# yinjunbo/IS-Fusion

Hardware: AMD Instinct MI355X
Metric: nuScenes frames/sec forward (0.075 voxel), LiDAR branch voxelize+spconv->BEV (higher is better)
Workload: dtype f32 (f16x3 split-precision MFMA, fp32 accumulate); 1 GPU; BASELINE configs[1]: isfusion_0075voxel LiDAR-only branch (dynamic voxelize + DynamicVFE + 21-layer SparseEncoder -> BEV [B,512,180,180]), synthetic nuScenes-shaped 300000-pt sweeps, batch=4/GPU, random-init weights, eval BN, fp32; points_per_frame=300000, batch_per_gpu=4, parallelism=dp1, collectives=none (1 rank)

## Files before the change

include/isf_hip.h:

```cpp
#ifndef ISF_HIP_H
#define ISF_HIP_H

#include <stddef.h>
#include <stdint.h>

#ifdef __cplusplus
extern "C" {
#endif

#define ISF_OK 0
#define ISF_ERR_ARG (-1)
#define ISF_ERR_HIP (-2)
#define ISF_ERR_NOMEM (-3)
#define ISF_ERR_UNSUPPORTED (-4)
#define ISF_ERR_CAPACITY (-5)

#define ISF_REDUCE_SUM 0
#define ISF_REDUCE_MEAN 1
#define ISF_REDUCE_MAX 2

#define ISF_CONV_SUBM 0
#define ISF_CONV_SPARSE 1

typedef void* isf_stream_t;
// ... 104 lines not shown
#define ISF_CONV_MODE_R4_ISSUE 131072
#define ISF_CONV_MODE_TWO_AHEAD 262144
#define ISF_CONV_MODE_CHUNK_SPLIT 524288
size_t isf_packed_filter16_bytes(int num_taps, int c_in, int c_out);
int isf_pack_filters_f16x3(const float* filters, int num_taps, int c_in, int c_out, void* packed16,
                           isf_stream_t stream);
int isf_pack_filters_dx(const float* filters_t, int num_taps, int c_in, int c_out, void* packed16, float* room,
                        isf_stream_t stream);
int isf_pack_filters_f16x3_transposed(const float* filters_t, int num_taps, int c_in, int c_out, void* packed16,
                                      isf_stream_t stream);
int isf_f32_to_split(const float* x, size_t num_elems, void* xs, isf_stream_t stream);
int isf_split_to_f32(const void* xs, size_t num_elems, float* x, isf_stream_t stream);
int isf_f32_to_half(const float* x, size_t num_elems, void* xh, isf_stream_t stream);
int isf_half_to_f32(const void* xh, size_t num_elems, float* x, isf_stream_t stream);
int isf_sparse_conv_forward_f16x3(const void* features_split, int num_in, int c_in, const void* packed16,
                                  int num_taps, int c_out, const int32_t* nbr, int nbr_stride, int num_out,
                                  const float* scale, const float* shift, const void* residual_split, int relu,
                                  void* out_split, int mode, isf_stream_t stream);
int isf_sparse_conv_tile_order(const int32_t* nbr, int nbr_stride, int num_taps, int num_out, int c_in, int c_out,
                               int mode, int32_t* work, int32_t* order, int* num_entries, isf_stream_t stream);
int isf_sparse_conv_forward_f16x3_ordered(const void* features_split, int num_in, int c_in, const void* packed16,
                                          int num_taps, int c_out, const int32_t* nbr, int nbr_stride, int num_out,
                                          const float* scale, const float* shift, const void* residual_split, int relu,
                                          void* out_split, int mode, const int32_t* order, isf_stream_t stream);
int isf_sparse_conv_tile_table(const int32_t* nbr, int nbr_stride, int num_taps, int num_out, int c_in, int c_out,
                               int mode, int32_t* scratch, int32_t* table, int* num_ints, isf_stream_t stream);
int isf_sparse_conv_forward_f16x3_tiled(const void* features_split, int num_in, int c_in, const void* packed16,
                                        int num_taps, int c_out, const int32_t* nbr, int nbr_stride, int num_out,
                                        const float* scale, const float* shift, const void* residual_split, int relu,
                                        void* out_split, int mode, const int32_t* table, isf_stream_t stream);
int isf_sparse_conv_tile_table_host(const int32_t* work, int num_groups, int part_groups, int parts, int cus, int wgs_per_cu,
                                    int groups_per_tile, int32_t* tiles, int* fits);
int isf_sparse_conv_trace(const void* features_split, int num_in, int c_in, const void* packed16, int num_taps,
                          int c_out, const int32_t* nbr, int nbr_stride, int num_out, const float* scale,
                          const float* shift, const void* residual_split, int relu, void* out_split,
                          const int32_t* order, long long* trace, int trace_capacity_blocks, int* grid_blocks,
                          isf_stream_t stream);
int isf_sparse_conv_phase_trace(const void* features_split, int num_in, int c_in, const void* packed16, int num_taps,
                                int c_out, const int32_t* nbr, int nbr_stride, int num_out, const float* scale,
                                const float* shift, const void* residual_split, int relu, void* out_split,
                                const int32_t* order, long long* trace, size_t trace_bytes, int* grid_blocks,
                                int* waves_per_block, int* dwords_per_wave, isf_stream_t stream);

int isf_sparse_conv_dma_trace(const void* features_split, int num_in, int c_in, const void* packed16, int num_taps,
                              int taps_per_line, int c_out, const int32_t* table, const uint32_t* mask, int nbr_stride,
                              int num_out, const float* scale, const float* shift, const void* residual_split, int relu,
                              void* out_split, long long* trace, int trace_capacity_blocks, int* grid_blocks,
                              isf_stream_t stream);
int isf_sparse_conv_dma_trace_parts(const void* features_split, int num_in, int c_in, const void* packed16, int num_taps,
                                    int taps_per_line, int c_out, const int32_t* table, const uint32_t* mask, int nbr_stride,
                                    int num_out, const float* scale, const float* shift, const void* residual_split, int relu,
                                    void* out_split, const int32_t* part_table, long long* trace, int trace_capacity_blocks,
                                    int* grid_blocks, isf_stream_t stream);
int isf_sparse_conv_part_table(const int32_t* table_nbr, const uint32_t* mask, int nbr_stride, int num_taps, int num_out,
                               int c_in, int c_out, int mode, int flags, int32_t* work, int work_capacity, int32_t* part_table,
                               int table_capacity, int* info, isf_stream_t stream);
int isf_sparse_conv_forward_parts(const void* features_split, int num_in, int c_in, const void* packed16, int num_taps,
                                  int taps_per_line, int c_out, const int32_t* table_nbr, const uint32_t* mask, int nbr_stride,
                                  int num_out, const float* scale, const float* shift, const void* residual_split, int relu,
                                  void* out_split, int mode, const int32_t* part_table, isf_stream_t stream);
int isf_sparse_conv_forward_dma(const void* features_split, int num_in, int c_in, const void* packed16, int num_taps,
                                int c_out, const int32_t* nbr, int nbr_stride, int num_out, const float* scale,
                                const float* shift, const void* residual_split, int relu, void* out_split, int mode,
                                const int32_t* order, isf_stream_t stream);
int isf_rulebook_to_lines(const int32_t* nbr, int nbr_stride, int num_taps, int taps_per_line, int num_out,
                          int32_t* lines, uint32_t* mask, int* not_consecutive_flag, isf_stream_t stream);
int isf_lines_to_rulebook(const int32_t* lines, const uint32_t* mask, int nbr_stride, int num_taps, int taps_per_line,
                          int32_t* nbr, isf_stream_t stream);
int isf_sparse_conv_forward_dma_lines(const void* features_split, int num_in, int c_in, const void* packed16, int num_taps,
                                      int taps_per_line, int c_out, const int32_t* lines, const uint32_t* mask,
                                      int nbr_stride, int num_out, const float* scale, const float* shift,
                                      const void* residual_split, int relu, void* out_split, int mode,
                                      isf_stream_t stream);
typedef struct isf_conv_cu_plan {
  const int32_t* group_masks;
  const int32_t* units;
  const int32_t* num_units;
  int max_units;
  int num_out;
  int variant;
  int cap;
} isf_conv_cu_plan;
int isf_sparse_conv_cu_plan_ints(int num_out, size_t* num_ints);
int isf_sparse_conv_cu_plan(const int32_t* nbr, int nbr_stride, int num_taps, int num_out, int32_t* plan_buf,
                            isf_conv_cu_plan* plan, isf_stream_t stream);
int isf_sparse_conv_forward_cu(const void* features_split, int num_in, int c_in, const void* packed16, int num_taps,
                               int c_out, const int32_t* nbr, int nbr_stride, int num_out, const float* scale,
                               const float* shift, const void* residual_split, int relu, void* out_split,
                               const isf_conv_cu_plan* plan, isf_stream_t stream);
int isf_sparse_conv_cu_plan_host(const int32_t* work, int num_groups, int cus, int32_t* units, int max_units,
                                 int* num_units);
int isf_sparse_conv_cu_max_units(int num_groups, int cus);
int isf_stage_unit_rows(void);
int isf_stage_unit_cap(void);
int isf_rulebook_stage_tables(const int32_t* nbr, int nbr_stride, int num_taps, uint16_t* slots, int32_t* ulist,
                              int32_t* ucount, isf_stream_t stream);
int isf_sparse_conv_forward_staged(const void* features_split, int num_in, int c_in, const void* packed16,
                                   int num_taps, int c_out, const uint16_t* slots, int nbr_stride,
                                   const int32_t* ulist, const int32_t* ucount, int num_out, const float* scale,
                                   const float* shift, const void* residual_split, int relu, void* out_split,
                                   int stage_rows, int mode, isf_stream_t stream);
int isf_sparse_to_dense_bev(const float* features, const int32_t* indices, int num_rows, int channels,
                            int batch_size, int D, int H, int W, float* out, isf_stream_t stream);

typedef struct isf_conv_layer {
  int conv_type;
// ... 509 lines not shown
```

is-fusion_amd/_lib.py:

```python
import ctypes
import os

_HERE = os.path.dirname(os.path.abspath(__file__))
LIB_PATH = os.path.join(_HERE, "libisf_hip.so")

c_int = ctypes.c_int
c_void_p = ctypes.c_void_p
c_float_p = ctypes.POINTER(ctypes.c_float)
c_int_p = ctypes.POINTER(ctypes.c_int)

ISF_OK = 0
REDUCE = {"sum": 0, "mean": 1, "max": 2}
CONV_SUBM, CONV_SPARSE = 0, 1


class ConvLayer(ctypes.Structure):
    _fields_ = [
        ("conv_type", c_int),
        ("ksize", c_int * 3), ("stride", c_int * 3), ("padding", c_int * 3),
        ("c_in", c_int), ("c_out", c_int),
        ("packed", c_void_p), ("packed16", c_void_p), ("scale", c_void_p), ("shift", c_void_p),
        ("relu", c_int), ("residual_from", c_int),
    ]

# ... 216 lines not shown
    "isf_ingroup_indices": (c_int, [c_void_p, c_int, c_void_p, c_void_p]),
    "isf_packed_window_block_bytes": (ctypes.c_size_t, [c_int]),
    "isf_pack_window_block": (c_int, [c_void_p, c_void_p, c_int, c_int, c_void_p, c_void_p]),
    "isf_window_block_forward": (c_int, [c_void_p, c_int, c_int, c_int, c_int, c_int, c_int, c_void_p, c_void_p,
                                         c_void_p, c_void_p, c_void_p, c_void_p, ctypes.c_float, c_void_p, c_void_p]),
    "isf_p2g_backward": (c_int, [c_void_p, c_int, c_int, c_void_p, c_int, c_int, c_int, c_int, c_int, c_int, c_void_p,
                                 c_int, c_int, c_int, c_void_p, c_void_p, c_void_p]),
    "isf_p2g_backward_det": (c_int, [c_void_p, c_int, c_int, c_void_p, c_int, c_int, c_int, c_int, c_int, c_int, c_void_p,
                                 c_int, c_int, c_int, c_void_p, c_void_p, c_void_p]),
    "isf_sparse_to_dense_bev": (c_int, [c_void_p, c_void_p, c_int, c_int, c_int, c_int, c_int, c_int,
                                        c_void_p, c_void_p]),
    "isf_sparse_encoder_forward": (c_int, [c_void_p, c_void_p, c_int, c_int, _I3,
                                           ctypes.POINTER(ConvLayer), c_int, c_void_p, _I4,
                                           ctypes.POINTER(EncoderStats), c_int, ctypes.POINTER(EncoderOptions),
                                           c_void_p]),
    "isf_lidar_branch_forward": (c_int, [c_void_p, ctypes.POINTER(ctypes.c_int64), c_int,
                                         ctypes.POINTER(VfeParams), _I3, ctypes.POINTER(ConvLayer), c_int,
                                         c_void_p, _I4, ctypes.POINTER(EncoderStats), c_int,
                                         ctypes.POINTER(EncoderOptions), c_void_p]),
    "isf_lidar_branch_forward_frames": (c_int, [ctypes.POINTER(c_void_p), ctypes.POINTER(ctypes.c_int64), c_int,
                                                ctypes.POINTER(VfeParams), _I3, ctypes.POINTER(ConvLayer), c_int,
                                                c_void_p, _I4, ctypes.POINTER(EncoderStats), c_int,
                                                ctypes.POINTER(EncoderOptions), c_void_p]),
    "isf_packed_linear_bytes": (ctypes.c_size_t, [c_int, c_int]),
    "isf_pack_linear": (c_int, [c_void_p, c_int, c_int, c_void_p, c_void_p]),
    "isf_pack_linear_transposed": (c_int, [c_void_p, c_int, c_int, c_void_p, c_void_p]),
    "isf_linear_forward": (c_int, [c_void_p, c_int, c_int, c_int, c_void_p, c_int, c_void_p, c_void_p, c_void_p,
                                   c_int, c_void_p, c_void_p, c_void_p, ctypes.c_float, c_void_p, c_int, c_int, c_int,
                                   c_int, c_void_p]),
    "isf_window_attention_forward": (c_int, [c_void_p, c_int, c_int, c_int, c_int, c_int, c_int, c_void_p,
                                             c_void_p]),
    "isf_attention_forward": (c_int, [c_void_p, c_int, c_void_p, c_void_p, c_int, c_int, c_int, c_int, c_int,
                                      c_int, c_void_p, c_int, c_void_p]),
    "isf_attention_forward_dropout": (c_int, [c_void_p, c_int, c_void_p, c_void_p, c_int, c_int, c_int, c_int, c_int,
                                              c_int, ctypes.c_float, ctypes.c_uint64, c_void_p, c_int, c_void_p]),
    "isf_channel_attention_forward": (c_int, [c_void_p, c_void_p, c_int, c_int, c_void_p, c_void_p]),
    "isf_channel_attention_backward": (c_int, [c_void_p, c_void_p, c_void_p, c_int, c_int, c_void_p, c_void_p, c_void_p]),
    "isf_p2g_forward": (c_int, [c_void_p, c_int, c_int, c_void_p, c_int, c_void_p, c_int, c_int, c_int, c_int,
                                c_int, c_void_p, c_int, c_int, c_int, c_void_p, c_void_p]),
    "isf_p2g_forward_split": (c_int, [c_void_p, c_int, c_int, c_void_p, c_int, c_void_p, c_int, c_int, c_int, c_int,
                                      c_int, c_void_p, c_int, c_int, c_int, c_void_p, c_void_p]),
    "isf_instance_topk": (c_int, [c_void_p, c_int, c_int, c_int, c_int, c_int, ctypes.c_uint, c_void_p, c_void_p,
                                  c_void_p, c_void_p]),
    "isf_msda_forward": (c_int, [c_void_p, c_void_p, c_void_p, c_void_p, c_int, c_int, c_int, c_int, c_int,
                                 c_int, c_int, c_void_p, c_void_p]),
    "isf_decode_boxes": (c_int, [c_void_p] * 8 + [c_int, c_int, c_int, c_int, ctypes.POINTER(ctypes.c_float)]
                         + [c_void_p] * 5),
    "isf_sparse_conv_dma_trace": (c_int, [c_void_p, c_int, c_int, c_void_p, c_int, c_int, c_int, c_void_p, c_void_p, c_int,
                                         c_int, c_void_p, c_void_p, c_void_p, c_int, c_void_p, c_void_p, c_int,
                                         ctypes.POINTER(c_int), c_void_p]),
    "isf_sparse_conv_dma_trace_parts": (c_int, [c_void_p, c_int, c_int, c_void_p, c_int, c_int, c_int, c_void_p, c_void_p,
                                               c_int, c_int, c_void_p, c_void_p, c_void_p, c_int, c_void_p, c_void_p,
                                               c_void_p, c_int, ctypes.POINTER(c_int), c_void_p]),
    "isf_sparse_conv_part_table": (c_int, [c_void_p, c_void_p, c_int, c_int, c_int, c_int, c_int, c_int, c_int, c_void_p,
                                           c_int, c_void_p, c_int, c_int * 4, c_void_p]),
    "isf_sparse_conv_forward_parts": (c_int, [c_void_p, c_int, c_int, c_void_p, c_int, c_int, c_int, c_void_p, c_void_p,
                                              c_int, c_int, c_void_p, c_void_p, c_void_p, c_int, c_void_p, c_int, c_void_p,
                                              c_void_p]),
    "isf_instance_gather": (c_int, [c_void_p, c_int, c_int, c_int, c_int] + [c_void_p] * 10),
    "isf_head_query_init": (c_int, [c_void_p, c_void_p, c_int, c_int, c_int, c_int, c_int] + [c_void_p] * 14),
    "isf_head_scatter_predictions": (c_int, [c_int, ctypes.POINTER(c_void_p), ctypes.POINTER(c_int),
                                            ctypes.POINTER(c_int), ctypes.POINTER(c_int), ctypes.POINTER(c_void_p),
                                            c_int, c_void_p, c_void_p, c_int, c_int, c_void_p]),
    "isf_assemble_points": (c_int, [c_void_p, ctypes.POINTER(Sweep), c_int, c_int, ctypes.POINTER(PointAug),
                                    ctypes.POINTER(ctypes.c_float), c_void_p, c_void_p,
                                    ctypes.POINTER(ctypes.c_int32), c_void_p]),
    "isf_image_prepass": (c_int, [c_void_p, c_void_p, c_int, c_void_p, c_void_p, c_int, c_int, c_void_p, c_void_p]),
    "isf_assemble_points_paste": (c_int, [c_void_p, ctypes.POINTER(Sweep), c_int, c_int, ctypes.POINTER(PointAug),
                                          ctypes.POINTER(ctypes.c_float), ctypes.POINTER(ctypes.c_float),
                                          ctypes.POINTER(ctypes.c_int32), c_void_p, c_void_p,
                                          ctypes.POINTER(ctypes.c_int32), c_void_p]),
    "isf_image_paste": (c_int, [c_void_p, c_void_p, c_int, c_void_p, c_int, c_int, c_int, ctypes.c_double,
                                ctypes.c_double, ctypes.c_float, c_void_p]),
    "isf_transpose_rulebook": (c_int, [c_void_p, c_int, c_int, c_int, c_int, c_void_p, c_int, c_void_p]),
    "isf_sparse_conv_backward_input": (c_int, [c_void_p, c_int, c_int, c_void_p, c_int, c_int, c_void_p, c_int, c_int,
                                               c_void_p, c_void_p]),
    "isf_sparse_conv_backward_filter": (c_int, [c_void_p, c_int, c_int, c_void_p, c_int, c_int, c_void_p, c_int,
                                                c_int, c_void_p, c_void_p]),
    "isf_bn1d_stats": (c_int, [c_void_p, c_int, c_int, c_void_p, c_void_p]),
    "isf_bn1d_apply": (c_int, [c_void_p, c_int, c_int, c_void_p, ctypes.c_float, c_void_p, c_void_p, ctypes.c_float,
                               ctypes.c_float, c_int, c_void_p, c_void_p, c_void_p, c_int, c_void_p, c_void_p, c_void_p]),
    "isf_bn1d_stats_pivot": (c_int, [c_void_p, c_int, c_int, c_void_p, c_void_p, c_void_p]),
    "isf_bn1d_apply_pivot": (c_int, [c_void_p, c_int, c_int, c_void_p, c_void_p, ctypes.c_float, c_void_p, c_void_p,
                                     ctypes.c_float, ctypes.c_float, c_int, c_void_p, c_void_p, c_void_p, c_int, c_void_p,
                                     c_void_p, c_void_p]),
    "isf_bn1d_apply_pivot_counted": (c_int, [c_void_p, c_int, c_int, c_void_p, c_void_p, ctypes.c_float, c_void_p, c_void_p,
                                             ctypes.c_float, ctypes.c_float, c_int, c_void_p, c_void_p, c_void_p, c_void_p,
                                             c_int, c_void_p, c_void_p, c_void_p]),
    "isf_bn1d_backward_sums": (c_int, [c_void_p, c_void_p, c_void_p, c_int, c_int, c_void_p, c_void_p, c_void_p]),
    "isf_bn1d_backward_apply": (c_int, [c_void_p, c_void_p, c_void_p, c_int, c_int, c_void_p, c_void_p, c_void_p,
                                        ctypes.c_float, c_void_p, c_void_p, c_void_p, c_void_p, c_void_p]),
    "isf_thin_linear_forward": (c_int, [c_void_p, c_void_p, c_void_p, c_void_p, c_int, c_int, c_int, c_void_p]),
    "isf_thin_linear_parts": (c_int, [c_int]),
    "isf_thin_linear_backward": (c_int, [c_void_p, c_void_p, c_void_p, c_void_p, c_void_p, c_void_p, c_void_p, c_int,
                                         c_int, c_int, c_void_p]),
    "isf_pair_list_capacity": (c_int, [c_int, c_int]),
    "isf_rulebook_pair_lists": (c_int, [c_void_p, c_int, c_int, c_int, c_int, c_void_p, c_void_p, c_void_p]),
    "isf_grad_to_split": (c_int, [c_void_p, ctypes.c_size_t, c_void_p, c_void_p, c_void_p]),
    "isf_grad_rescale": (c_int, [c_void_p, ctypes.c_size_t, c_void_p, c_void_p, c_void_p]),
    "isf_split_to_f32_scaled": (c_int, [c_void_p, ctypes.c_size_t, c_void_p, c_void_p, c_void_p]),
    "isf_split_to_f32_scaled2": (c_int, [c_void_p, ctypes.c_size_t, c_void_p, c_void_p, c_void_p, c_void_p]),
    "isf_sparse_conv_backward_filter_f16x3": (c_int, [c_void_p, c_int, c_int, c_void_p, c_int, c_int, c_void_p, c_void_p,
                                                      c_int, c_int, c_void_p, c_void_p, c_int, c_void_p]),
    "isf_msda_backward": (c_int, [c_void_p] * 5 + [c_int] * 7 + [c_void_p] * 4),
    "isf_gather_cells_backward": (c_int, [c_void_p, c_void_p, c_int, c_int, c_int, c_int, c_int, c_void_p, c_void_p]),
    "isf_msda_backward_det": (c_int, [c_void_p] * 5 + [c_int] * 7 + [c_void_p] * 4),
# ... 173 lines not shown
```

is-fusion_amd/csrc/isf_spconv16.h:

```cpp
#pragma once
#include "isf_common.h"

namespace isf {

typedef _Float16 h8 __attribute__((ext_vector_type(8)));
typedef float f32x4 __attribute__((ext_vector_type(4)));
typedef float f32x8 __attribute__((ext_vector_type(8)));

static constexpr int kMaxTaps = 27;

static constexpr int kConvModeNarrowTiles = 64;
static constexpr int kConvModeTileTable = 1024;
static constexpr int kConvModePartTable = 16384;
static constexpr int kConvModeTileBits = ISF_CONV_MODE_UNIFORM_TILES | kConvModeTileTable | kConvModePartTable;

static constexpr bool conv_mode_is_production(int m) {
  return m == 0 || m == ISF_CONV_MODE_F16 || m == ISF_CONV_MODE_NO_SHARING || m == ISF_CONV_MODE_F16_STORAGE;
}
static constexpr bool conv_mode_is_knockout(int m) {
  return m == ISF_CONV_MODE_NO_GATHER || m == ISF_CONV_MODE_NO_WEIGHTS || m == (ISF_CONV_MODE_NO_GATHER | ISF_CONV_MODE_NO_WEIGHTS) ||
         m == ISF_CONV_MODE_NO_LOOP;
}
static constexpr int kConvIssueOpts = ISF_CONV_MODE_STAGGER | ISF_CONV_MODE_R4_ISSUE | ISF_CONV_MODE_TWO_AHEAD | ISF_CONV_MODE_CHUNK_SPLIT;
static constexpr int kConvOptsForward = ISF_CONV_MODE_UNIFORM_TILES | kConvIssueOpts | kConvModeNarrowTiles | ISF_CONV_MODE_ONE_BLOCK_4W |
                                        ISF_CONV_MODE_ONE_BLOCK_8W | ISF_CONV_MODE_DEEP;
static constexpr int kConvOptsOrdered = ISF_CONV_MODE_UNIFORM_TILES | kConvIssueOpts;
static constexpr int kConvOptsTiled = 0;
static constexpr int kConvOptsDma = ISF_CONV_MODE_UNIFORM_TILES;
static constexpr int kConvOptsStaged = ISF_CONV_MODE_UNIFORM_TILES;

static constexpr int kKernF16 = ISF_CONV_MODE_F16, kKernNoGather = ISF_CONV_MODE_NO_GATHER, kKernNoWeights = ISF_CONV_MODE_NO_WEIGHTS,
                     kKernNoLoop = ISF_CONV_MODE_NO_LOOP, kKernNoSharing = ISF_CONV_MODE_NO_SHARING, kKernF16Rows = ISF_CONV_MODE_F16_ROWS,
                     kKernStagger = ISF_CONV_MODE_STAGGER, kKernR4Issue = ISF_CONV_MODE_R4_ISSUE, kKernTwoAhead = ISF_CONV_MODE_TWO_AHEAD,
                     kKernChunkSplit = ISF_CONV_MODE_CHUNK_SPLIT;
static constexpr int kKernTrace = 512;
static constexpr int kKernPhaseTrace = 2048;
static constexpr int conv_kern_bits(int base) { return conv_mode_is_production(base) || conv_mode_is_knockout(base) ? base : -1; }

inline bool sparse_conv_f16x3_supported(int c_in, int c_out) {
  return (c_in == 32 || c_in == 64 || c_in == 128 || c_in == 256) &&
         (c_out == 32 || c_out == 64 || c_out == 128 || c_out == 256);
}
inline bool sparse_conv_dma_supported(int c_in, int c_out) { return (c_in == 32 || c_in == 64) && (c_out == 32 || c_out == 64); }
inline bool sparse_conv_deep_supported(int c_in, int c_out) { return (c_in == 128 || c_in == 256) && (c_out == 128 || c_out == 256); }

static constexpr int kConv16NW = 4, kConv16RG = 2;
inline bool conv16_wide_shape(int c_out, int n_out) { return c_out == 128 && n_out >= 8 * 256; }
inline int conv16_small_rows_256(int cus) { return 96 * cus; }
inline int conv16_small_rows_wide(int cus) { return 256 * cus; }

enum { kConv16Tile = 0, kConv16Deep = 1 };
struct Conv16Choice {
  int backend;
  int nt, rg, nw;
  int kern;
  bool uniform_tiles;
  bool drop_order;
};
static constexpr int kConvModeOneBlock = ISF_CONV_MODE_ONE_BLOCK_4W | ISF_CONV_MODE_ONE_BLOCK_8W;
static constexpr int kConvModeShapeBits = kConvModeNarrowTiles | ISF_CONV_MODE_DEEP | kConvIssueOpts | kConvModeOneBlock;
inline int conv16_choose(int c_in, int c_out, int n_out, int mode, bool has_rowmap, int cus, Conv16Choice* out) {
  if (!sparse_conv_f16x3_supported(c_in, c_out)) return ISF_ERR_UNSUPPORTED;
  const bool deep = sparse_conv_deep_supported(c_in, c_out), nt8 = c_out >= 128;
  const bool wide = conv16_wide_shape(c_out, n_out), small256 = deep && c_out == 256 && n_out <= conv16_small_rows_256(cus);
  *out = Conv16Choice{kConv16Tile, nt8 ? 8 : c_out / 16, kConv16RG, kConv16NW, 0, false, false};
  int m = mode & ~(kConvModeNarrowTiles | ISF_CONV_MODE_DEEP);
  const auto left = [&m](int bits) { return (m & ~kConvModeTileBits) == bits; };
  const auto variant = [out](int nw, int kern) { out->nw = nw; out->kern = kern; return ISF_OK; };
  if (deep && c_out == 256 && left(ISF_CONV_MODE_CHUNK_SPLIT)) { out->rg = small256 ? 1 : 2; return variant(4, kKernChunkSplit); }
  m &= ~ISF_CONV_MODE_CHUNK_SPLIT;
  if (deep && c_out == 256 && !has_rowmap && (m & kConvModeOneBlock) && left(m & kConvModeOneBlock)) {
    const bool w8 = (m & ISF_CONV_MODE_ONE_BLOCK_8W) != 0;
    *out = Conv16Choice{kConv16Tile, 16, w8 ? 1 : 2, w8 ? 8 : 4, 0, w8, true};
    return ISF_OK;
  }
  m &= ~kConvModeOneBlock;
  if (deep && !wide && left(ISF_CONV_MODE_TWO_AHEAD)) return variant(4, kKernTwoAhead);
  m &= ~ISF_CONV_MODE_TWO_AHEAD;
  if (nt8 && left(ISF_CONV_MODE_R4_ISSUE)) return variant(wide ? 8 : 4, kKernR4Issue);
  m &= ~ISF_CONV_MODE_R4_ISSUE;
  if (nt8 && left(ISF_CONV_MODE_STAGGER)) return variant(wide ? 8 : 4, kKernStagger);
  m &= ~ISF_CONV_MODE_STAGGER;
  if (const int base = m & ~kConvModeTileBits) {
    if (conv_kern_bits(base) < 0) return ISF_ERR_ARG;
    const bool production = base == ISF_CONV_MODE_F16_STORAGE || base == ISF_CONV_MODE_NO_SHARING;
    return variant(production && wide ? 8 : 4, conv_kern_bits(base));
  }
  const bool small_wide = wide && n_out <= conv16_small_rows_wide(cus);
  if (small_wide || small256) out->rg = 1;
// ... 360 lines not shown
```

is-fusion_amd/csrc/isf_spconv_dma.hip:

```cpp
#include "isf_spconv_launch.h"


namespace isf {

#ifndef ISF_DMA_KNOCKOUT
#define ISF_DMA_KNOCKOUT 0
#endif
#ifndef ISF_DMA_EARLY_B
#define ISF_DMA_EARLY_B 1
#endif
__device__ uint4 g_zero_line[8];

constexpr int kDmaTraceWords = 16;
__device__ __forceinline__ unsigned long long dma_shader_clock() {
  unsigned long long t;
  asm volatile("s_memtime %0\n\ts_waitcnt lgkmcnt(0)" : "=s"(t) : : "memory");
  return t;
}

template <int NT, int NW, int RG = 2>
struct ConvDmaSmem {
  static constexpr int TM = 16 * RG * NW;
  static constexpr int bbuf_bytes = 2 * NT * 2048;
  static constexpr int transit_bytes = NW * RG * 2048;
  static constexpr int epi_bytes = NW * Conv16Epi<NT, RG>::wave_bytes;
  static constexpr int main_bytes = bbuf_bytes + transit_bytes;
  static constexpr int bytes = main_bytes > epi_bytes ? main_bytes : epi_bytes;
};

template <int CIN, int NT, int NW, int MODE, int RG = 2, bool LINES = false>
__global__ __launch_bounds__(64 * NW) void spconv_dma_kernel(
    const uint4* __restrict__ xs, const int32_t* __restrict__ nbr, const uint32_t* __restrict__ lmask, int nx,
    int nbr_stride, const uint4* __restrict__ wpk,
    const float* __restrict__ w_inv_scale, int K, int cout, const float* __restrict__ scale,
    const float* __restrict__ shift, const uint4* __restrict__ residual, uint4* __restrict__ ys, int n_out, int relu,
    Conv16Plan plan, const int32_t* __restrict__ order,
    const int32_t* __restrict__ rowmap ,
    long long* __restrict__ trace ) {
  constexpr bool HALF = (MODE & kKernF16) != 0, F16IO = (MODE & kKernF16Rows) != 0, TRACE = (MODE & kKernTrace) != 0;
  long long t_entry = 0, t_pro = 0, t_loop = 0;
  unsigned long long c_wait = 0, c_bar = 0, c_issue = 0, c_mul = 0, c_rd = 0, c_adv = 0;
  if (TRACE) t_entry = wall_clock64();
  static_assert(!F16IO || HALF, "f16 storage implies single-pass f16 arithmetic");
  using S = ConvDmaSmem<NT, NW, RG>;
  constexpr int NTHR = 64 * NW, TM = S::TM, WR = 16 * RG;
  constexpr int NCH = CIN / 32, CH8 = CIN / 8, BN = 16 * NT;
  extern __shared__ __attribute__((aligned(16))) char smem[];
  uint4* bbuf = reinterpret_cast<uint4*>(smem);
  int* misc = reinterpret_cast<int*>(smem);

  const int tid = threadIdx.x, lane = tid & 63;
  const int wave = __builtin_amdgcn_readfirstlane(tid >> 6);
  const int col = lane & 15, kg = lane >> 4;
  const int ncb = cout / BN;
  int cb, row0, row_end;
  bool half_tile;
  if (!conv16_tile_of_block(ncb, plan, TM, n_out, cb, row0, row_end, half_tile, order)) return;
  const int ntiles_total = cout >> 4;
  const int row0w = row0 + wave * (half_tile ? WR / 2 : WR);
  const int wrows = half_tile ? WR / 2 : WR;

  unsigned rgm[RG];
#pragma unroll
  for (int rg = 0; rg < RG; ++rg) rgm[rg] = 0u;
  if constexpr (LINES) {
    const int row = row0w + lane;
    const unsigned mrow = (lane < wrows && row < row_end) ? lmask[row] : 0u;
#pragma unroll
    for (int k = 0; k < kMaxTaps; ++k) {
      const unsigned long long m = __ballot((mrow >> k) & 1u);
#pragma unroll
      for (int rg = 0; rg < RG; ++rg) rgm[rg] |= (((m >> (16 * rg)) & 0xffffull) ? 1u : 0u) << k;
    }
  } else {
    int tmp[kMaxTaps];
    const int row = row0w + lane;
    const bool live = lane < wrows && row < row_end;
#pragma unroll
    for (int k = 0; k < kMaxTaps; ++k) {
      tmp[k] = -1;
      if (k < K && live) tmp[k] = nbr[(size_t)k * nbr_stride + row];
    }
#pragma unroll
    for (int k = 0; k < kMaxTaps; ++k) {
      const unsigned long long m = __ballot(tmp[k] >= 0);
#pragma unroll
      for (int rg = 0; rg < RG; ++rg) rgm[rg] |= (((m >> (16 * rg)) & 0xffffull) ? 1u : 0u) << k;
    }
  }
  unsigned wmask = 0u;
#pragma unroll
  for (int rg = 0; rg < RG; ++rg) {
    rgm[rg] = __builtin_amdgcn_readfirstlane(rgm[rg]);
    wmask |= rgm[rg];
  }
  if (lane == 0) misc[wave] = (int)wmask;
  __syncthreads();
  unsigned wg_mask = 0;
#pragma unroll
  for (int w = 0; w < NW; ++w) wg_mask |= (unsigned)misc[w];
  wg_mask = __builtin_amdgcn_readfirstlane(wg_mask);
  __syncthreads();
  const int nsteps = __popc(wg_mask) * NCH;

  f32x4 acc[RG][NT];
#pragma unroll
  for (int rg = 0; rg < RG; ++rg)
#pragma unroll
    for (int nt = 0; nt < NT; ++nt) acc[rg][nt] = f32x4{0.f, 0.f, 0.f, 0.f};

  const int grow_l = lane >> 2;
  const int gpiece = ((lane & 3) - (grow_l >> 2)) & 3;
  const int rpos = 4 * col + ((kg + (col >> 2)) & 3);
  const unsigned bbuf_addr = __builtin_amdgcn_readfirstlane(lds_addr(bbuf));
  const uint4* transit = reinterpret_cast<const uint4*>(smem + S::bbuf_bytes) + wave * (RG * 128);
  const unsigned transit_addr = __builtin_amdgcn_readfirstlane(lds_addr(transit));
  const uint4* zero = g_zero_line;

  auto load_idx = [&](int tap, int (&idx)[RG]) {
#pragma unroll
    for (int rg = 0; rg < RG; ++rg) {
      const int row = row0w + rg * 16 + grow_l;
      idx[rg] = -1;
      if (((rgm[rg] >> tap) & 1u) && row < row_end) idx[rg] = nbr[(size_t)tap * nbr_stride + row];
    }
  };
  unsigned mg[RG];
  int base_cur[RG], base_nxt[RG];
  int line_cur = -1;
#pragma unroll
  for (int rg = 0; rg < RG; ++rg) {
    mg[rg] = 0u;
    base_cur[rg] = base_nxt[rg] = -1;
    if constexpr (LINES) {
      const int row = row0w + rg * 16 + grow_l;
      if (rgm[rg] && row < row_end) mg[rg] = lmask[row];
    }
  }
  auto line_of = [&](int tap) -> int { return nx == 3 ? (tap * 43) >> 7 : tap; };
  auto load_line = [&](int line, int (&base)[RG]) {
#pragma unroll
    for (int rg = 0; rg < RG; ++rg) {
      const int row = row0w + rg * 16 + grow_l;
      const unsigned lbits = ((nx == 3 ? 7u : 1u) << (line * nx));
      base[rg] = -1;
      if ((mg[rg] & lbits) && row < row_end) base[rg] = nbr[(size_t)line * nbr_stride + row];
    }
  };
  auto line_idx = [&](int tap, int (&idx)[RG]) {
    const unsigned first = (unsigned)(line_of(tap) * nx);
    const unsigned below = ((1u << tap) - 1u) & ~((1u << first) - 1u);
#pragma unroll
    for (int rg = 0; rg < RG; ++rg)
      idx[rg] = ((mg[rg] >> tap) & 1u) ? base_cur[rg] + __popc(mg[rg] & below) : -1;
  };
  auto issue_A = [&](int tap, int ch, const int (&idx)[RG]) {
    if constexpr ((ISF_DMA_KNOCKOUT & 1) != 0) return;
#pragma unroll
    for (int rg = 0; rg < RG; ++rg) {
      if ((rgm[rg] >> tap) & 1u) {
        const uint4* src = zero + gpiece;
        if (idx[rg] >= 0)
          src = F16IO ? xs + (size_t)idx[rg] * CH8 + ch * 4 + gpiece
                      : xs + ((size_t)idx[rg] * CH8 + ch * 4) * 2 + gpiece;
        glds16(src, transit_addr + (unsigned)(rg * 2) * 1024u);
        if (!HALF) glds16(src + 4, transit_addr + (unsigned)(rg * 2 + 1) * 1024u);
      }
    }
  };
  constexpr int PW = NT * 128 / NW;
  auto stage_B = [&](int tap, int ch, int buf) {
    if constexpr ((ISF_DMA_KNOCKOUT & 2) != 0) return;
    if constexpr (HALF ? (PW == 128 || PW == 256) : (PW == 64 || PW == 128 || PW == 256)) {
      const uint4* srun = wpk + (((size_t)tap * NCH + ch) * ntiles_total + cb * NT) * 128 + wave * PW + lane;
      const unsigned drun = bbuf_addr + (unsigned)(buf * (NT * 128) + wave * PW) * 16u;
      if constexpr (HALF) glds16_run_hi<PW / 64>(srun, drun);
      else glds16_run<PW / 64>(srun, drun);
      return;
    }
    const uint4* src = wpk + (((size_t)tap * NCH + ch) * ntiles_total + cb * NT) * 128;
    const unsigned dst = bbuf_addr + (unsigned)(buf * (NT * 128)) * 16u;
#pragma unroll
    for (int i = 0; i < (NT * 128 + NTHR - 1) / NTHR; ++i) {
      const int base = i * NTHR + wave * 64;
      if (base < NT * 128 && !(HALF && ((base >> 6) & 1))) glds16(src + base + lane, dst + (unsigned)base * 16u);
    }
  };

  unsigned rem = wg_mask;
  int tap = -1, ch = NCH - 1;
  int idx_cur[RG], idx_nxt[RG];
#pragma unroll
  for (int rg = 0; rg < RG; ++rg) idx_cur[rg] = idx_nxt[rg] = -1;
  auto advance = [&]() {
    if (++ch == NCH) {
      ch = 0;
      tap = __ffs(rem) - 1;
      rem &= rem - 1;
      if constexpr (LINES) {
        const int line = line_of(tap);
        if (line != line_cur) {
          line_cur = line;
#pragma unroll
          for (int rg = 0; rg < RG; ++rg) base_cur[rg] = base_nxt[rg];
          const unsigned later = (line + 1) * nx < 32 ? rem & ~((1u << ((line + 1) * nx)) - 1u) : 0u;
          if (later) load_line(line_of(__ffs(later) - 1), base_nxt);
        }
        line_idx(tap, idx_cur);
      } else {
#pragma unroll
        for (int rg = 0; rg < RG; ++rg) idx_cur[rg] = idx_nxt[rg];
        if (rem) load_idx(__ffs(rem) - 1, idx_nxt);
      }
    }
  };
  if (TRACE) t_pro = wall_clock64();
  if (nsteps > 0) {
    if constexpr (LINES) load_line(line_of(__ffs(rem) - 1), base_nxt);
    else load_idx(__ffs(rem) - 1, idx_nxt);
    advance();
    issue_A(tap, ch, idx_cur);
    stage_B(tap, ch, 0);
  }
  for (int s = 0; s < nsteps; ++s) {
    const int tap_s = tap;
    unsigned long long c0 = 0, c1 = 0, c2 = 0, c3 = 0;
    if (TRACE) c0 = dma_shader_clock();
    __builtin_amdgcn_s_waitcnt(0x0F70);
    if (TRACE) c1 = dma_shader_clock();
    if constexpr ((ISF_DMA_KNOCKOUT & 8) == 0)
      __syncthreads();
    if (TRACE) c2 = dma_shader_clock();
    uint4 a_cur[RG][2];
#pragma unroll
    for (int rg = 0; rg < RG; ++rg) {
      a_cur[rg][0] = make_uint4(0, 0, 0, 0);
      a_cur[rg][1] = make_uint4(0, 0, 0, 0);
      if ((rgm[rg] >> tap_s) & 1u) {
        a_cur[rg][0] = transit[(rg * 2) * 64 + rpos];
        if (!HALF) a_cur[rg][1] = transit[(rg * 2 + 1) * 64 + rpos];
      }
    }
    const uint4* b = bbuf + (s & 1) * (NT * 128) + lane;
    uint4 bhu_n = b[0], blu_n = make_uint4(0, 0, 0, 0);
    if (!HALF) blu_n = b[64];
    const bool more = s + 1 < nsteps;
#if ISF_DMA_EARLY_B
    unsigned long long ca = 0, cb = 0;
    if (TRACE) ca = dma_shader_clock();
    if (more) {
      advance();
      stage_B(tap, ch, (s + 1) & 1);
    }
    if (TRACE) cb = dma_shader_clock();
    __builtin_amdgcn_s_waitcnt(0xC07F);
    if (more) issue_A(tap, ch, idx_cur);
    if (TRACE) {
      c_rd += ca - c2;
      c_adv += cb - ca;
    }
#else
    __builtin_amdgcn_s_waitcnt(0xC07F);
    if (more) {
      advance();
      issue_A(tap, ch, idx_cur);
      stage_B(tap, ch, (s + 1) & 1);
    }
#endif
    if (TRACE) {
      c3 = dma_shader_clock();
      c_wait += c1 - c0;
      c_bar += c2 - c1;
      c_issue += c3 - c2;
    }
    if (((wmask >> tap_s) & 1u) && (ISF_DMA_KNOCKOUT & 4) == 0) {
      bool need[RG];
#pragma unroll
      for (int rg = 0; rg < RG; ++rg) need[rg] = (rgm[rg] >> tap_s) & 1u;
#pragma unroll
      for (int nt = 0; nt < NT; ++nt) {
        const uint4 bhu = bhu_n, blu = blu_n;
        if (nt + 1 < NT) {
          bhu_n = b[((nt + 1) * 2 + 0) * 64];
          if (!HALF) blu_n = b[((nt + 1) * 2 + 1) * 64];
        }
        const h8 bh = *reinterpret_cast<const h8*>(&bhu);
        const h8 bl = *reinterpret_cast<const h8*>(&blu);
#pragma unroll
        for (int rg = 0; rg < RG; ++rg) {
          if (need[rg]) {
            const h8 ah = *reinterpret_cast<const h8*>(&a_cur[rg][0]);
            const h8 al = *reinterpret_cast<const h8*>(&a_cur[rg][1]);
            if (!HALF) {
              acc[rg][nt] = __builtin_amdgcn_mfma_f32_16x16x32_f16(al, bh, acc[rg][nt], 0, 0, 0);
              acc[rg][nt] = __builtin_amdgcn_mfma_f32_16x16x32_f16(ah, bl, acc[rg][nt], 0, 0, 0);
            }
            acc[rg][nt] = __builtin_amdgcn_mfma_f32_16x16x32_f16(ah, bh, acc[rg][nt], 0, 0, 0);
          }
        }
      }
    }
    if (TRACE) c_mul += dma_shader_clock() - c3;
  }
  __builtin_amdgcn_s_waitcnt(0x0F70);
  __syncthreads();
  if (TRACE) t_loop = wall_clock64();

  float* tile_l = reinterpret_cast<float*>(smem) + wave * (Conv16Epi<NT, RG>::wave_bytes / 4);
  conv16_epilogue<NT, RG, F16IO>(acc, tile_l, lane, row0w, cb * BN, cout, *w_inv_scale, scale, shift, residual, ys,
                                 row_end, relu, half_tile ? RG / 2 : RG, rowmap);
  if (TRACE) {
    __syncthreads();
    if (tid == 0) {
      unsigned hw_id, xcc_id;
      asm volatile("s_getreg_b32 %0, hwreg(HW_REG_HW_ID)" : "=s"(hw_id));
      asm volatile("s_getreg_b32 %0, hwreg(HW_REG_XCC_ID)" : "=s"(xcc_id));
      long long* t = trace + (size_t)blockIdx.x * kDmaTraceWords;
      t[0] = t_entry; t[1] = t_pro; t[2] = t_loop; t[3] = wall_clock64();
      t[4] = nsteps; t[5] = hw_id; t[6] = xcc_id; t[7] = (long long)row0 | ((long long)half_tile << 32);
      t[8] = (long long)c_wait; t[9] = (long long)c_bar; t[10] = (long long)c_issue; t[11] = (long long)c_mul;
      t[12] = (long long)c_rd; t[13] = (long long)c_adv; t[14] = 0; t[15] = 0;
    }
  }
}

template <int CIN, int NT, int MODE, bool LINES, int NW = 4, int RG = 2>
static int launch_dma(const ConvCall& c, Conv16LaunchInfo* query) {
  using S = ConvDmaSmem<NT, NW, RG>;
  auto kern = spconv_dma_kernel<CIN, NT, NW, MODE, RG, LINES>;
  static ConvSlots slots;
  ISF_TRY(conv_kernel_slots(slots, reinterpret_cast<const void*>(kern), 64 * NW, S::bytes, S::bytes));
  const Conv16Plan plan = conv16_launch_plan(c, S::TM, c.c_out / (16 * NT), slots, true, query);
  if (query) return ISF_OK;
  const ConvWeights w = conv_weights(c);
  hipLaunchKernelGGL(kern, dim3(conv16_grid_blocks(plan)), dim3(64 * NW), S::bytes, c.st, reinterpret_cast<const uint4*>(c.xs),
                     c.nbr, c.lmask, c.nx, c.nbr_stride, w.wpk, w.winv, c.K, c.c_out, c.scale, c.shift,
                     reinterpret_cast<const uint4*>(c.residual), reinterpret_cast<uint4*>(c.ys), c.n_out, c.relu, plan, c.order,
                     c.rowmap, c.trace);
  ISF_LAUNCH_CHECK();
  return ISF_OK;
}

template <int CIN, int NT, int MODE>
static int launch_dma_table(const ConvCall& c, bool lines, Conv16LaunchInfo* query) {
  return lines ? launch_dma<CIN, NT, MODE, true>(c, query) : launch_dma<CIN, NT, MODE, false>(c, query);
}
template <int CIN, int NT>
static int dispatch_dma(const ConvCall& c, bool lines, Conv16LaunchInfo* query) {
  const int mode = c.mode & ~kConvModePartTable, base = mode & ~kConvOptsDma;
  switch (base == kKernTrace ? base : conv_kern_bits(base)) {
    case kKernTrace: return launch_dma_table<CIN, NT, kKernTrace>(c, lines, query);
    case 0: return launch_dma_table<CIN, NT, 0>(c, lines, query);
    case kKernF16: return launch_dma_table<CIN, NT, kKernF16>(c, lines, query);
    case kKernF16Rows | kKernF16: return launch_dma_table<CIN, NT, kKernF16Rows | kKernF16>(c, lines, query);
  }
  ISF_REQUIRE(false, ISF_ERR_ARG, "sparse_conv_dma: mode %d (0, 1, 257, +32)", mode);
}

static int run_dma(const ConvCall& c, bool lines, Conv16LaunchInfo* query) {
  if (c.c_in == 32) return c.c_out == 32 ? dispatch_dma<32, 2>(c, lines, query) : dispatch_dma<32, 4>(c, lines, query);
  return c.c_out == 32 ? dispatch_dma<64, 2>(c, lines, query) : dispatch_dma<64, 4>(c, lines, query);
}

static int check_dma(const ConvCall& c) {
  ISF_TRY(conv_check_problem("sparse_conv_dma", c.c_in, c.c_out, sparse_conv_dma_supported(c.c_in, c.c_out), c.K, c.nbr_stride,
                             c.n_out));
  ISF_REQUIRE(!c.lmask || ((c.nx == 1 || c.nx == 3) && c.K % c.nx == 0), ISF_ERR_ARG, "sparse_conv_dma: %d taps in lines of %d",
              c.K, c.nx);
  return ISF_OK;
}

int sparse_conv_forward_dma_impl(const ConvCall& c) {
  if (c.n_out <= 0) return ISF_OK;
  ISF_TRY(check_dma(c));
  return run_dma(c, c.lmask != nullptr, nullptr);
}

int conv_dma_launch_info(bool lines, int c_in, int c_out, int n_out, int mode, Conv16LaunchInfo* info) {
  ISF_REQUIRE(sparse_conv_dma_supported(c_in, c_out), ISF_ERR_UNSUPPORTED, "sparse_conv_dma: (Cin,Cout)=(%d,%d) not built",
              c_in, c_out);
  ConvCall q;
  q.c_in = c_in; q.c_out = c_out; q.n_out = n_out; q.mode = mode;
  return run_dma(q, lines, info);
}

static int trace_dma(const char* entry, const ConvCall& c, int blocks, int trace_capacity_blocks, int* grid_blocks) {
  ISF_REQUIRE(blocks <= trace_capacity_blocks, ISF_ERR_ARG, "%s: the launch has %d workgroups, the trace buffer holds %d", entry,
              blocks, trace_capacity_blocks);
  *grid_blocks = blocks;
  return sparse_conv_forward_dma_impl(c);
}

}

extern "C" {

int isf_sparse_conv_forward_dma(const void* features_split, int num_in, int c_in, const void* packed16, int num_taps,
                                int c_out, const int32_t* nbr, int nbr_stride, int num_out, const float* scale,
                                const float* shift, const void* residual_split, int relu, void* out_split, int mode,
                                const int32_t* order, isf_stream_t stream) {
  isf::ConvCall c = isf::conv_call(features_split, c_in, packed16, num_taps, c_out, nbr, nbr_stride, num_out, scale, shift,
                                   residual_split, relu, out_split, mode, isf::as_stream(stream));
  c.order = order;
  bool run;
  ISF_TRY(isf::conv_entry_check("sparse_conv_forward_dma", c, num_in, true, nbr != nullptr, &run));
  return run ? isf::sparse_conv_forward_dma_impl(c) : ISF_OK;
}

int isf_sparse_conv_forward_dma_lines(const void* features_split, int num_in, int c_in, const void* packed16, int num_taps,
                                      int taps_per_line, int c_out, const int32_t* lines, const uint32_t* mask,
                                      int nbr_stride, int num_out, const float* scale, const float* shift,
                                      const void* residual_split, int relu, void* out_split, int mode,
                                      isf_stream_t stream) {
  isf::ConvCall c = isf::conv_call(features_split, c_in, packed16, num_taps, c_out, lines, nbr_stride, num_out, scale, shift,
                                   residual_split, relu, out_split, mode, isf::as_stream(stream));
  c.lmask = mask;
  c.nx = taps_per_line;
  bool run;
  ISF_TRY(isf::conv_entry_check("sparse_conv_forward_dma_lines", c, num_in, true, lines && mask, &run));
  return run ? isf::sparse_conv_forward_dma_impl(c) : ISF_OK;
}

int isf_sparse_conv_dma_trace(const void* features_split, int num_in, int c_in, const void* packed16, int num_taps,
                              int taps_per_line, int c_out, const int32_t* table, const uint32_t* mask, int nbr_stride,
                              int num_out, const float* scale, const float* shift, const void* residual_split, int relu,
                              void* out_split, long long* trace, int trace_capacity_blocks, int* grid_blocks,
                              isf_stream_t stream) {
  ISF_REQUIRE(num_in >= 0 && num_out > 0 && features_split && packed16 && table && out_split && trace && grid_blocks &&
                  trace_capacity_blocks > 0 && ((scale == nullptr) == (shift == nullptr)), ISF_ERR_ARG,
              "sparse_conv_dma_trace: bad arguments");
  isf::ConvCall c = isf::conv_call(features_split, c_in, packed16, num_taps, c_out, table, nbr_stride, num_out, scale, shift,
                                   residual_split, relu, out_split, isf::kKernTrace, isf::as_stream(stream));
  c.lmask = mask;
  c.nx = taps_per_line;
  c.trace = trace;
  ISF_TRY(isf::check_dma(c));
  isf::Conv16LaunchInfo info;
  ISF_TRY(isf::conv16_launch_info(mask ? isf::kConvKernelDmaLines : isf::kConvKernelDma, c_in, c_out, num_out, c.mode, &info));
  return isf::trace_dma("sparse_conv_dma_trace", c, 8 * (info.full + info.half) , trace_capacity_blocks,
                        grid_blocks);
}

int isf_sparse_conv_dma_trace_parts(const void* features_split, int num_in, int c_in, const void* packed16, int num_taps,
                                    int taps_per_line, int c_out, const int32_t* table, const uint32_t* mask, int nbr_stride,
                                    int num_out, const float* scale, const float* shift, const void* residual_split, int relu,
                                    void* out_split, const int32_t* part_table, long long* trace, int trace_capacity_blocks,
                                    int* grid_blocks, isf_stream_t stream) {
  ISF_REQUIRE(num_in >= 0 && num_out > 0 && features_split && packed16 && table && out_split && trace && grid_blocks &&
// ... 20 lines not shown
```

Baseline: 1081 frames/s.

## Hand-schedule f16x3 MFMA multiply step in inline asm for DMA sparse conv

Replaces the compiler-generated multiply step of the DMA sparse-conv kernel (NT=2, RG=2, fp32 split mode) with a hand-written inline-asm block that interleaves ds_read_b128 of the B tile with staggered lgkmcnt waits and the three split-precision MFMAs per row group. It branches on scalar row-group needs. It also makes neighbor-index prefetch unconditional by clamping the row and always loading, removing branches. It raises the launch-bounds occupancy hint for that variant and keeps the old path selectable through a runtime toggle. The risks are a fixed s_nop pad, register-pressure changes from the occupancy hint, and an extra index load when no later tap exists.

```diff
diff --git a/include/isf_hip.h b/include/isf_hip.h
--- a/include/isf_hip.h
+++ b/include/isf_hip.h
@@ -180,6 +180,7 @@
                                     int num_out, const float* scale, const float* shift, const void* residual_split, int relu,
                                     void* out_split, const int32_t* part_table, long long* trace, int trace_capacity_blocks,
                                     int* grid_blocks, isf_stream_t stream);
+int isf_sparse_conv_dma_old_step(int on);
 int isf_sparse_conv_part_table(const int32_t* table_nbr, const uint32_t* mask, int nbr_stride, int num_taps, int num_out,
                                int c_in, int c_out, int mode, int flags, int32_t* work, int work_capacity, int32_t* part_table,
                                int table_capacity, int* info, isf_stream_t stream);
diff --git a/is-fusion_amd/_lib.py b/is-fusion_amd/_lib.py
--- a/is-fusion_amd/_lib.py
+++ b/is-fusion_amd/_lib.py
@@ -292,6 +292,7 @@
     "isf_sparse_conv_dma_trace_parts": (c_int, [c_void_p, c_int, c_int, c_void_p, c_int, c_int, c_int, c_void_p, c_void_p,
                                                c_int, c_int, c_void_p, c_void_p, c_void_p, c_int, c_void_p, c_void_p,
                                                c_void_p, c_int, ctypes.POINTER(c_int), c_void_p]),
+    "isf_sparse_conv_dma_old_step": (c_int, [c_int]),
     "isf_sparse_conv_part_table": (c_int, [c_void_p, c_void_p, c_int, c_int, c_int, c_int, c_int, c_int, c_int, c_void_p,
                                            c_int, c_void_p, c_int, c_int * 4, c_void_p]),
     "isf_sparse_conv_forward_parts": (c_int, [c_void_p, c_int, c_int, c_void_p, c_int, c_int, c_int, c_void_p, c_void_p,
diff --git a/is-fusion_amd/csrc/isf_spconv16.h b/is-fusion_amd/csrc/isf_spconv16.h
--- a/is-fusion_amd/csrc/isf_spconv16.h
+++ b/is-fusion_amd/csrc/isf_spconv16.h
@@ -35,6 +35,7 @@
                      kKernChunkSplit = ISF_CONV_MODE_CHUNK_SPLIT;
 static constexpr int kKernTrace = 512;
 static constexpr int kKernPhaseTrace = 2048;
+static constexpr int kKernOldStep = 1024;
 static constexpr int conv_kern_bits(int base) { return conv_mode_is_production(base) || conv_mode_is_knockout(base) ? base : -1; }
 
 inline bool sparse_conv_f16x3_supported(int c_in, int c_out) {
diff --git a/is-fusion_amd/csrc/isf_spconv_dma.hip b/is-fusion_amd/csrc/isf_spconv_dma.hip
--- a/is-fusion_amd/csrc/isf_spconv_dma.hip
+++ b/is-fusion_amd/csrc/isf_spconv_dma.hip
@@ -1,13 +1,22 @@
 #include "isf_spconv_launch.h"
-
+#include "isf_spconv_dma_mult.h"
+
+#include <atomic>
 
 namespace isf {
+
+typedef int i32x4 __attribute__((ext_vector_type(4)));
+
+static std::atomic<int> g_dma_old_step{0};
 
 #ifndef ISF_DMA_KNOCKOUT
 #define ISF_DMA_KNOCKOUT 0
 #endif
 #ifndef ISF_DMA_EARLY_B
 #define ISF_DMA_EARLY_B 1
+#endif
+#ifndef ISF_DMA_NEW_STEP
+#define ISF_DMA_NEW_STEP 3
 #endif
 __device__ uint4 g_zero_line[8];
 
@@ -28,8 +37,11 @@
   static constexpr int bytes = main_bytes > epi_bytes ? main_bytes : epi_bytes;
 };
 
+static constexpr bool conv_dma_asm_multiply(int nt, int rg, int mode) {
+  return !(mode & (kKernOldStep | kKernF16)) && (ISF_DMA_NEW_STEP & 1) && rg == 2 && nt == 2 && (ISF_DMA_KNOCKOUT & 4) == 0;
+}
 template <int CIN, int NT, int NW, int MODE, int RG = 2, bool LINES = false>
-__global__ __launch_bounds__(64 * NW) void spconv_dma_kernel(
+__global__ __launch_bounds__(64 * NW, conv_dma_asm_multiply(NT, RG, MODE) ? 5 : 1) void spconv_dma_kernel(
     const uint4* __restrict__ xs, const int32_t* __restrict__ nbr, const uint32_t* __restrict__ lmask, int nx,
     int nbr_stride, const uint4* __restrict__ wpk,
     const float* __restrict__ w_inv_scale, int K, int cout, const float* __restrict__ scale,
@@ -38,6 +50,9 @@
     const int32_t* __restrict__ rowmap ,
     long long* __restrict__ trace ) {
   constexpr bool HALF = (MODE & kKernF16) != 0, F16IO = (MODE & kKernF16Rows) != 0, TRACE = (MODE & kKernTrace) != 0;
+  constexpr bool OLD = (MODE & kKernOldStep) != 0;
+  constexpr bool ASMM = conv_dma_asm_multiply(NT, RG, MODE);
+  constexpr bool OLD_IDX = OLD || !(ISF_DMA_NEW_STEP & 2);
   long long t_entry = 0, t_pro = 0, t_loop = 0;
   unsigned long long c_wait = 0, c_bar = 0, c_issue = 0, c_mul = 0, c_rd = 0, c_adv = 0;
   if (TRACE) t_entry = wall_clock64();
@@ -121,8 +136,12 @@
 #pragma unroll
     for (int rg = 0; rg < RG; ++rg) {
       const int row = row0w + rg * 16 + grow_l;
-      idx[rg] = -1;
-      if (((rgm[rg] >> tap) & 1u) && row < row_end) idx[rg] = nbr[(size_t)tap * nbr_stride + row];
+      if constexpr (OLD_IDX) {
+        idx[rg] = -1;
+        if (((rgm[rg] >> tap) & 1u) && row < row_end) idx[rg] = nbr[(size_t)tap * nbr_stride + row];
+      } else {
+        idx[rg] = nbr[(size_t)tap * nbr_stride + (row < row_end ? row : row_end - 1)];
+      }
     }
   };
   unsigned mg[RG];
@@ -142,9 +161,13 @@
 #pragma unroll
     for (int rg = 0; rg < RG; ++rg) {
       const int row = row0w + rg * 16 + grow_l;
-      const unsigned lbits = ((nx == 3 ? 7u : 1u) << (line * nx));
-      base[rg] = -1;
-      if ((mg[rg] & lbits) && row < row_end) base[rg] = nbr[(size_t)line * nbr_stride + row];
+      if constexpr (OLD_IDX) {
+        const unsigned lbits = ((nx == 3 ? 7u : 1u) << (line * nx));
+        base[rg] = -1;
+        if ((mg[rg] & lbits) && row < row_end) base[rg] = nbr[(size_t)line * nbr_stride + row];
+      } else {
+        base[rg] = nbr[(size_t)line * nbr_stride + (row < row_end ? row : row_end - 1)];
+      }
     }
   };
   auto line_idx = [&](int tap, int (&idx)[RG]) {
@@ -192,6 +215,13 @@
   int idx_cur[RG], idx_nxt[RG];
 #pragma unroll
   for (int rg = 0; rg < RG; ++rg) idx_cur[rg] = idx_nxt[rg] = -1;
+  auto rotate = [&](int (&cur)[RG], const int (&nxt)[RG]) {
+#pragma unroll
+    for (int rg = 0; rg < RG; ++rg) {
+      if constexpr (OLD_IDX) cur[rg] = nxt[rg];
+      else asm volatile("v_mov_b32 %0, %1" : "=v"(cur[rg]) : "v"(nxt[rg]) : "memory");
+    }
+  };
   auto advance = [&]() {
     if (++ch == NCH) {
       ch = 0;
@@ -201,16 +231,22 @@
         const int line = line_of(tap);
         if (line != line_cur) {
           line_cur = line;
-#pragma unroll
-          for (int rg = 0; rg < RG; ++rg) base_cur[rg] = base_nxt[rg];
+          rotate(base_cur, base_nxt);
           const unsigned later = (line + 1) * nx < 32 ? rem & ~((1u << ((line + 1) * nx)) - 1u) : 0u;
-          if (later) load_line(line_of(__ffs(later) - 1), base_nxt);
+          if constexpr (OLD_IDX) {
+            if (later) load_line(line_of(__ffs(later) - 1), base_nxt);
+          } else {
+            load_line(later ? line_of(__ffs(later) - 1) : line, base_nxt);
+          }
         }
         line_idx(tap, idx_cur);
       } else {
-#pragma unroll
-        for (int rg = 0; rg < RG; ++rg) idx_cur[rg] = idx_nxt[rg];
-        if (rem) load_idx(__ffs(rem) - 1, idx_nxt);
+        rotate(idx_cur, idx_nxt);
+        if constexpr (OLD_IDX) {
+          if (rem) load_idx(__ffs(rem) - 1, idx_nxt);
+        } else {
+          load_idx(rem ? __ffs(rem) - 1 : tap, idx_nxt);
+        }
       }
     }
   };
@@ -273,7 +309,21 @@
       c_bar += c2 - c1;
       c_issue += c3 - c2;
     }
-    if (((wmask >> tap_s) & 1u) && (ISF_DMA_KNOCKOUT & 4) == 0) {
+    if constexpr (ASMM) {
+      if ((wmask >> tap_s) & 1u) {
+        const unsigned vb = bbuf_addr + (unsigned)((s & 1) * (NT * 128) + lane) * 16u;
+        const int n0 = (int)((rgm[0] >> tap_s) & 1u), n1 = (int)((rgm[RG - 1] >> tap_s) & 1u);
+        const i32x4 a0h = *reinterpret_cast<const i32x4*>(&a_cur[0][0]), a0l = *reinterpret_cast<const i32x4*>(&a_cur[0][1]);
+        const i32x4 a1h = *reinterpret_cast<const i32x4*>(&a_cur[RG - 1][0]),
+                    a1l = *reinterpret_cast<const i32x4*>(&a_cur[RG - 1][1]);
+        i32x4 xh, xl, yh, yl;
+        asm volatile(ISF_DM_TEXT
+                     : [c00] "+v"(acc[0][0]), [c01] "+v"(acc[0][NT - 1]), [c10] "+v"(acc[RG - 1][0]), [c11] "+v"(acc[RG - 1][NT - 1]),
+                       [xh] "=&v"(xh), [xl] "=&v"(xl), [yh] "=&v"(yh), [yl] "=&v"(yl)
+                     : [a0h] "v"(a0h), [a0l] "v"(a0l), [a1h] "v"(a1h), [a1l] "v"(a1l), [vb] "v"(vb), [n0] "s"(n0), [n1] "s"(n1)
+                     : "scc", "memory");
+      }
+    } else if (((wmask >> tap_s) & 1u) && (ISF_DMA_KNOCKOUT & 4) == 0) {
       bool need[RG];
 #pragma unroll
       for (int rg = 0; rg < RG; ++rg) need[rg] = (rgm[rg] >> tap_s) & 1u;
@@ -348,11 +398,16 @@
 template <int CIN, int NT>
 static int dispatch_dma(const ConvCall& c, bool lines, Conv16LaunchInfo* query) {
   const int mode = c.mode & ~kConvModePartTable, base = mode & ~kConvOptsDma;
+  const bool old = g_dma_old_step.load(std::memory_order_relaxed) != 0;
   switch (base == kKernTrace ? base : conv_kern_bits(base)) {
     case kKernTrace: return launch_dma_table<CIN, NT, kKernTrace>(c, lines, query);
-    case 0: return launch_dma_table<CIN, NT, 0>(c, lines, query);
-    case kKernF16: return launch_dma_table<CIN, NT, kKernF16>(c, lines, query);
-    case kKernF16Rows | kKernF16: return launch_dma_table<CIN, NT, kKernF16Rows | kKernF16>(c, lines, query);
+    case 0: return old ? launch_dma_table<CIN, NT, kKernOldStep>(c, lines, query) : launch_dma_table<CIN, NT, 0>(c, lines, query);
+    case kKernF16:
+      return old ? launch_dma_table<CIN, NT, kKernOldStep | kKernF16>(c, lines, query)
+                 : launch_dma_table<CIN, NT, kKernF16>(c, lines, query);
+    case kKernF16Rows | kKernF16:
+      return old ? launch_dma_table<CIN, NT, kKernOldStep | kKernF16Rows | kKernF16>(c, lines, query)
+                 : launch_dma_table<CIN, NT, kKernF16Rows | kKernF16>(c, lines, query);
   }
   ISF_REQUIRE(false, ISF_ERR_ARG, "sparse_conv_dma: mode %d (0, 1, 257, +32)", mode);
 }
@@ -394,6 +449,8 @@
 }
 
 extern "C" {
+
+int isf_sparse_conv_dma_old_step(int on) { return isf::g_dma_old_step.exchange(on != 0 ? 1 : 0); }
 
 int isf_sparse_conv_forward_dma(const void* features_split, int num_in, int c_in, const void* packed16, int num_taps,
                                 int c_out, const int32_t* nbr, int nbr_stride, int num_out, const float* scale,
diff --git a/is-fusion_amd/csrc/isf_spconv_dma_mult.h b/is-fusion_amd/csrc/isf_spconv_dma_mult.h
--- /dev/null
+++ b/is-fusion_amd/csrc/isf_spconv_dma_mult.h
@@ -0,0 +1,35 @@
+#pragma once
+
+#define ISF_DM_MF(C, A, B) "v_mfma_f32_16x16x32_f16 " C ", " A ", " B ", " C "\n\t"
+#define ISF_DM_RD(REG, OFF) "ds_read_b128 " REG ", %[vb] offset:" #OFF "\n\t"
+#define ISF_DM_WAIT(N) "s_waitcnt lgkmcnt(" #N ")\n\t"
+#define ISF_DM_READS ISF_DM_RD("%[xh]", 0) ISF_DM_RD("%[yh]", 2048) ISF_DM_RD("%[xl]", 1024) ISF_DM_RD("%[yl]", 3072)
+#define ISF_DM_PAD "s_nop 11\n\t"
+
+#define ISF_DM_BOTH                                                                                                     \
+  ISF_DM_READS                                                                                                          \
+  ISF_DM_WAIT(3) ISF_DM_MF("%[c00]", "%[a0l]", "%[xh]") ISF_DM_MF("%[c10]", "%[a1l]", "%[xh]")                          \
+  ISF_DM_WAIT(2) ISF_DM_MF("%[c01]", "%[a0l]", "%[yh]") ISF_DM_MF("%[c11]", "%[a1l]", "%[yh]")                          \
+  ISF_DM_WAIT(1) ISF_DM_MF("%[c00]", "%[a0h]", "%[xl]") ISF_DM_MF("%[c10]", "%[a1h]", "%[xl]")                          \
+  ISF_DM_WAIT(0) ISF_DM_MF("%[c01]", "%[a0h]", "%[yl]") ISF_DM_MF("%[c11]", "%[a1h]", "%[yl]")                          \
+  ISF_DM_MF("%[c00]", "%[a0h]", "%[xh]") ISF_DM_MF("%[c10]", "%[a1h]", "%[xh]")                                         \
+  ISF_DM_MF("%[c01]", "%[a0h]", "%[yh]") ISF_DM_MF("%[c11]", "%[a1h]", "%[yh]") ISF_DM_PAD
+#define ISF_DM_ONE(R)                                                                                                   \
+  ISF_DM_READS                                                                                                          \
+  ISF_DM_WAIT(3) ISF_DM_MF("%[c" #R "0]", "%[a" #R "l]", "%[xh]") ISF_DM_WAIT(2) ISF_DM_MF("%[c" #R "1]", "%[a" #R "l]", "%[yh]") \
+  ISF_DM_WAIT(1) ISF_DM_MF("%[c" #R "0]", "%[a" #R "h]", "%[xl]") ISF_DM_WAIT(0) ISF_DM_MF("%[c" #R "1]", "%[a" #R "h]", "%[yl]") \
+  ISF_DM_MF("%[c" #R "0]", "%[a" #R "h]", "%[xh]") ISF_DM_MF("%[c" #R "1]", "%[a" #R "h]", "%[yh]") ISF_DM_PAD
+
+#define ISF_DM_TEXT                                                                                                     \
+  "s_cmp_eq_u32 %[n0], 0\n\t"                                                                                           \
+  "s_cbranch_scc1 LDM1_%=\n\t"                                                                                          \
+  "s_cmp_eq_u32 %[n1], 0\n\t"                                                                                           \
+  "s_cbranch_scc1 LDM0_%=\n\t"                                                                                          \
+  ISF_DM_BOTH                                                                                                           \
+  "s_branch LDME_%=\n\t"                                                                                                \
+  "LDM0_%=:\n\t"                                                                                                        \
+  ISF_DM_ONE(0)                                                                                                         \
+  "s_branch LDME_%=\n\t"                                                                                                \
+  "LDM1_%=:\n\t"                                                                                                        \
+  ISF_DM_ONE(1)                                                                                                         \
+  "LDME_%=:\n\t"
```

Measured after the change: 1092 frames/s (median of 4 runs). 1.01x the previous value.
